# plai-group/latent-flexible-video-diffusion-modeling

Hardware: NVIDIA B200
Metric: denoiser frame-steps/sec (sampling) (higher is better)
Workload: dtype bf16

## Files before the change

### include/fdm_b200.h

```cpp
#ifndef FDM_B200_H_
#define FDM_B200_H_

#include <stddef.h>
#include <stdint.h>

#ifdef __cplusplus
extern "C" {
#endif

#define FDM_ABI_VERSION 2

enum { FDM_F32 = 0, FDM_BF16 = 1 };

enum {
  FDM_OK = 0,
  FDM_ERR_BAD_ARG = -1,
  FDM_ERR_UNSUPPORTED = -2,
  FDM_ERR_CUDA = -3,
  FDM_ERR_NO_DEVICE = -4
};

int fdm_abi_version(void);
const char* fdm_status_string(int status);
const char* fdm_last_cuda_error(void);
// ... 18 lines not shown
  const float* bias;
  const float* resid;
  float* y_f32;
  void* y_op;
  double* stats;
  int32_t N, Hin, Win, C0, C1, Cout;
  int32_t ksize, stride, upsample;
  int32_t a_dtype, op_dtype, out_nchw, engine;
  int32_t resid_norm;
  int32_t rn_T;
  float rn_eps;
  const float* rn_tstats;
  const double* rn_stats;
  const float* rn_gamma;
  const float* rn_beta;
} fdm_conv_args;
int fdm_conv(const fdm_conv_args* a, void* stream);

typedef struct {
  const void* xa;
  const float* xb;
  const double* stats_a;
  const double* stats_b;
  const float* gamma;
  const float* beta;
  const float* film;
  void* out_op;
  float* out_f32;
  void* raw_op;
  int32_t N, HW, Ca, Cb, T;
// ... 337 lines not shown
```

### latent-flexible-video-diffusion-modeling_b200/csrc/conv_simt.cu

```cuda
#include "common.cuh"

namespace fdm {

constexpr int BM = 64, BN = 64, BK = 16, NT = 256;

struct ConvParams {
  const void* a0;
  const float* w0;
  const void* a1;
  const float* w1;
  const float* bias;
  const float* resid;
  float* y_f32;
  void* y_op;
  double* stats;
  int N, Hin, Win, C0, C1, Cout, Ho, Wo;
  int ksize, stride, upsample, out_nchw;
  int M;
};

template <typename AT, typename OT>
__global__ void __launch_bounds__(NT) conv_simt_kernel(ConvParams p) {
  pdl_wait();
  __shared__ __align__(16) float As[BK][BM + 4];
// ... 202 lines not shown
  return check_launch();
}

}

extern "C" int fdm_conv(const fdm_conv_args* a, void* stream) {
  using namespace fdm;
  FDM_REQUIRE(a != nullptr && a->a0 != nullptr && a->w0 != nullptr, FDM_ERR_BAD_ARG);
  FDM_REQUIRE(a->N > 0 && a->Hin > 0 && a->Win > 0 && a->C0 > 0 && a->Cout > 0, FDM_ERR_BAD_ARG);
  FDM_REQUIRE(a->ksize == 1 || a->ksize == 3, FDM_ERR_UNSUPPORTED);
  FDM_REQUIRE(a->stride == 1 || a->stride == 2, FDM_ERR_UNSUPPORTED);
  FDM_REQUIRE(!(a->upsample && a->stride != 1), FDM_ERR_UNSUPPORTED);
  FDM_REQUIRE((a->a1 == nullptr) == (a->w1 == nullptr), FDM_ERR_BAD_ARG);
  FDM_REQUIRE(a->y_f32 != nullptr || a->y_op != nullptr, FDM_ERR_BAD_ARG);
  FDM_REQUIRE(!(a->out_nchw && a->y_f32 == nullptr), FDM_ERR_BAD_ARG);
  cudaStream_t st = reinterpret_cast<cudaStream_t>(stream);
  if (a->engine == FDM_CONV_TC) {
    if (a->out_nchw && a->ksize == 3) {
      const int rh = conv_head_launch(a, st);
      if (rh != FDM_ERR_UNSUPPORTED) return rh;
    }
    const int rc = (a->ksize == 3 || a->C0 >= 256) ? conv_halo_launch(a, st) : FDM_ERR_UNSUPPORTED;
    return rc == FDM_ERR_UNSUPPORTED ? conv_tc_launch(a, st) : rc;
  }
  if (a->engine == FDM_CONV_TC_TAP) return conv_tc_launch(a, st);
  FDM_REQUIRE(a->engine == FDM_CONV_SIMT, FDM_ERR_BAD_ARG);
  FDM_REQUIRE(a->resid_norm == 0, FDM_ERR_UNSUPPORTED);
  return conv_simt_launch(a, st);
}
```

### latent-flexible-video-diffusion-modeling_b200/csrc/conv_tc.cu

```cuda
#include "tc_common.cuh"
#include <mutex>

namespace fdm {

constexpr int TC_BM = 128;
constexpr int TC_BK = 64;
constexpr int TC_THREADS = 192;
constexpr int A_TILE_BYTES = TC_BM * TC_BK * 2;

struct TcParams {
  const float* bias;
  const float* resid;
  float* y_f32;
  __nv_bfloat16* y_op;
  double* stats;
  int M, HWo, Wo, Ho, Cout;
  int wbox, hbox, nbox;
  int taps, ksize, pad, stride;
  int kchunks0, kchunks1;
  int klast0, klast1;
  int out_nchw;
  int stages;
  int nr;
  int a_slot;
  int stage_bytes;
  int resid_norm, rn_T;
  float rn_eps;
  double rn_inv_cnt;
  const float* rn_tstats;
  const double* rn_stats;
  const float* rn_gamma;
  const float* rn_beta;
};

constexpr int TC_MAX_STAGES = 8;
constexpr int TC_STG_ROW = 36;

template <int BN>
struct TcSmem {
  static constexpr int B_TILE_BYTES = BN * TC_BK * 2;
  static constexpr int STAGE_BYTES = A_TILE_BYTES + B_TILE_BYTES;
  static constexpr int TMEM_COLS = BN < 32 ? 32 : BN;
  static constexpr int EXTRA_BYTES = 1024;
  static_assert(STAGE_BYTES >= 4 * 32 * TC_STG_ROW * 4, "one stage must hold the epilogue staging");
};

template <int BN, bool RN>
__global__ void __launch_bounds__(TC_THREADS, RN ? 3 : 0) conv_tc_kernel(const __grid_constant__ CUtensorMap ta0,
                                                            const __grid_constant__ CUtensorMap tw0,
                                                            const __grid_constant__ CUtensorMap ta1,
                                                            const __grid_constant__ CUtensorMap tw1, const TcParams p) {
  using S = TcSmem<BN>;
  extern __shared__ uint8_t smem_raw[];
  uint8_t* smem = reinterpret_cast<uint8_t*>((reinterpret_cast<uintptr_t>(smem_raw) + 1023) & ~uintptr_t(1023));
  __shared__ __align__(8) uint64_t full_bar[TC_MAX_STAGES];
  __shared__ __align__(8) uint64_t empty_bar[TC_MAX_STAGES];
  __shared__ __align__(8) uint64_t tmem_full_bar;
  __shared__ uint32_t tmem_base_slot;
  __shared__ __align__(16) float4 rn_tab[RN ? 4 : 1][2][2][RN ? 32 : 1];

  const int warp = threadIdx.x >> 5, lane = threadIdx.x & 31;
  const int mt = blockIdx.x, n_off = blockIdx.y * BN;
  const int m0 = mt * TC_BM;
  const int iters0 = (p.taps / p.nr) * p.kchunks0;
  const int iters = iters0 + p.kchunks1;
  const int stages = p.stages;
  constexpr int B_TAP_BYTES = BN * 128;

  if (warp == 0 && lane == 0) {
    asm volatile("prefetch.tensormap [%0];" ::"l"(&ta0) : "memory");
    asm volatile("prefetch.tensormap [%0];" ::"l"(&tw0) : "memory");
    if (p.kchunks1) {
      asm volatile("prefetch.tensormap [%0];" ::"l"(&ta1) : "memory");
      asm volatile("prefetch.tensormap [%0];" ::"l"(&tw1) : "memory");
// ... 93 lines not shown
        }
        umma_commit(&empty_bar[stage]);
        }
        __syncwarp();
        if (++stage == stages) { stage = 0; phase ^= 1; }
      }
      if (elect_one_sync()) umma_commit(&tmem_full_bar);
      __syncwarp();
    }
  } else {
    const int g = warp & 3;
    float* stg = reinterpret_cast<float*>(smem) + g * 32 * TC_STG_ROW;
    const int sub = lane >> 3, cq = (lane & 7) * 4;
    const int m_w = m0 + g * 32;
    const bool two_frames = p.HWo < 32;
    int rn_n[2] = {0, 0}, rn_b[2] = {0, 0};
    if (RN) {
      rn_n[0] = min(m_w, p.M - 1) / p.HWo;
      rn_n[1] = two_frames ? min(m_w + 16, p.M - 1) / p.HWo : rn_n[0];
      rn_b[0] = rn_n[0] / p.rn_T;
      rn_b[1] = rn_n[1] / p.rn_T;
      if (p.resid_norm == 3) {
        const int col = n_off + 4 * lane;
#pragma unroll
        for (int hh = 0; hh < 2; ++hh) {
          float4 mu = make_float4(0.f, 0.f, 0.f, 0.f), ad = mu;
          if ((hh == 0 || two_frames) && col < p.Cout && 4 * lane < BN && m_w + hh * 16 < p.M) {
            const float4 gm = __ldg(reinterpret_cast<const float4*>(p.rn_gamma + col));
            const float4 bt = __ldg(reinterpret_cast<const float4*>(p.rn_beta + col));
            const double2* st = reinterpret_cast<const double2*>(p.rn_stats + ((size_t)rn_n[hh] * p.Cout + col) * 2);
            const double2 s0 = st[0], s1_ = st[1], s2_ = st[2], s3 = st[3];
            const double mean = (s0.x + s1_.x + s2_.x + s3.x) * p.rn_inv_cnt;
            const double var = fmax((s0.y + s1_.y + s2_.y + s3.y) * p.rn_inv_cnt - mean * mean, 0.0);
            const float mf = (float)mean, rs = rsqrtf((float)var + p.rn_eps);
            mu = make_float4(gm.x * rs, gm.y * rs, gm.z * rs, gm.w * rs);
            ad = make_float4(bt.x - mf * mu.x, bt.y - mf * mu.y, bt.z - mf * mu.z, bt.w - mf * mu.w);
          }
          rn_tab[g][hh][0][lane] = mu;
          rn_tab[g][hh][1][lane] = ad;
        }
        __syncwarp();
      }
    }
    mbar_wait(&tmem_full_bar, 0);
    tcgen05_fence_after();
    const bool direct = BN >= 32 && p.y_f32 == nullptr && p.y_op != nullptr && p.resid == nullptr && p.stats == nullptr &&
                        !p.out_nchw && (p.Cout & 31) == 0;
#pragma unroll 1
    for (int c = 0; c < BN; c += 32) {
      uint32_t v[32];
      tmem_ld_32x32b_x32(tmem_base + ((uint32_t)(g * 32) << 16) + c, v);
      if (direct) {
        uint8_t* sb = reinterpret_cast<uint8_t*>(stg);
        const bool cols_ok = n_off + c < p.Cout;
#pragma unroll
        for (int q = 0; q < 32; q += 8) {
          float4 b0 = make_float4(0.f, 0.f, 0.f, 0.f), b1 = b0;
          if (p.bias != nullptr && cols_ok) {
            b0 = __ldg(reinterpret_cast<const float4*>(p.bias + n_off + c + q));
            b1 = __ldg(reinterpret_cast<const float4*>(p.bias + n_off + c + q + 4));
          }
// ... 70 lines not shown
            const int grp = (c + cq) >> 2;
#pragma unroll
            for (int hh = 0; hh < 2; ++hh) {
              const float4 mu = rn_tab[g][two_frames ? hh : 0][0][grp], ad = rn_tab[g][two_frames ? hh : 0][1][grp];
#pragma unroll
              for (int i = 4 * hh; i < 4 * hh + 4; ++i) {
                res[i].x = fmaf(res[i].x, mu.x, ad.x);
                res[i].y = fmaf(res[i].y, mu.y, ad.y);
                res[i].z = fmaf(res[i].z, mu.z, ad.z);
                res[i].w = fmaf(res[i].w, mu.w, ad.w);
              }
            }
          }
        }
        float s1[2][4], s2[2][4];
#pragma unroll
        for (int hh = 0; hh < 2; ++hh)
#pragma unroll
          for (int q = 0; q < 4; ++q) s1[hh][q] = s2[hh][q] = 0.f;
#pragma unroll
        for (int i = 0; i < 8; ++i) {
          const int row = i * 4 + sub;
          const int m = m_w + row;
          const float4 a = *reinterpret_cast<const float4*>(stg + row * TC_STG_ROW + cq);
          const float o[4] = {a.x + bias.x + res[i].x, a.y + bias.y + res[i].y, a.z + bias.z + res[i].z, a.w + bias.w + res[i].w};
          if (m < p.M && col_ok) {
#pragma unroll
            for (int q = 0; q < 4; ++q) { s1[i >> 2][q] += o[q]; s2[i >> 2][q] = fmaf(o[q], o[q], s2[i >> 2][q]); }
            const size_t off = (size_t)m * p.Cout + col;
            if (p.y_f32 != nullptr) *reinterpret_cast<float4*>(p.y_f32 + off) = make_float4(o[0], o[1], o[2], o[3]);
            if (p.y_op != nullptr) OpType<__nv_bfloat16>::store4(p.y_op + off, make_float4(o[0], o[1], o[2], o[3]));
          }
        }
        if (p.stats != nullptr) {
#pragma unroll
          for (int hh = 0; hh < 2; ++hh)
#pragma unroll
            for (int q = 0; q < 4; ++q) {
              s1[hh][q] += __shfl_xor_sync(0xffffffffu, s1[hh][q], 8);
              s2[hh][q] += __shfl_xor_sync(0xffffffffu, s2[hh][q], 8);
              s1[hh][q] += __shfl_xor_sync(0xffffffffu, s1[hh][q], 16);
              s2[hh][q] += __shfl_xor_sync(0xffffffffu, s2[hh][q], 16);
            }
          if (sub == 0 && col_ok) {
            if (two_frames) {
#pragma unroll
// ... 2 lines not shown
                if (mseg < p.M) {
                  double* dst = p.stats + ((size_t)(mseg / p.HWo) * p.Cout + col) * 2;
#pragma unroll
                  for (int q = 0; q < 4; ++q) {
                    atomicAdd(dst + 2 * q, (double)s1[hh][q]);
                    atomicAdd(dst + 2 * q + 1, (double)s2[hh][q]);
                  }
                }
              }
            } else if (m_w < p.M) {
              double* dst = p.stats + ((size_t)(m_w / p.HWo) * p.Cout + col) * 2;
#pragma unroll
              for (int q = 0; q < 4; ++q) {
                atomicAdd(dst + 2 * q, (double)(s1[0][q] + s1[1][q]));
                atomicAdd(dst + 2 * q + 1, (double)(s2[0][q] + s2[1][q]));
              }
            }
          }
        }
      }
      __syncwarp();
    }
  }
  tcgen05_fence_before();
  __syncthreads();
  if (warp == 2) {
    tcgen05_fence_after();
    asm volatile("tcgen05.dealloc.cta_group::1.sync.aligned.b32 %0, %1;" ::"r"(tmem_base), "n"(S::TMEM_COLS));
  }
}
// ... 21 lines not shown
  return enc(m, CU_TENSOR_MAP_DATA_TYPE_BFLOAT16, 4, const_cast<void*>(ptr), dims, strides, box, estr, CU_TENSOR_MAP_INTERLEAVE_NONE,
             CU_TENSOR_MAP_SWIZZLE_128B, CU_TENSOR_MAP_L2_PROMOTION_L2_128B, CU_TENSOR_MAP_FLOAT_OOB_FILL_NONE) == CUDA_SUCCESS;
}

static bool encode_w(CUtensorMap* m, const void* ptr, int taps, int co_pad, int ci_pad, int bn, int box_taps) {
  EncodeTiledFn enc = get_tensormap_encoder();
  if (!enc) return false;
  cuuint64_t dims[3] = {(cuuint64_t)ci_pad, (cuuint64_t)co_pad, (cuuint64_t)taps};
  cuuint64_t strides[2] = {(cuuint64_t)ci_pad * 2, (cuuint64_t)co_pad * ci_pad * 2};
  cuuint32_t box[3] = {(cuuint32_t)TC_BK, (cuuint32_t)bn, (cuuint32_t)box_taps};
  cuuint32_t estr[3] = {1, 1, 1};
  return enc(m, CU_TENSOR_MAP_DATA_TYPE_BFLOAT16, 3, const_cast<void*>(ptr), dims, strides, box, estr, CU_TENSOR_MAP_INTERLEAVE_NONE,
             CU_TENSOR_MAP_SWIZZLE_128B, CU_TENSOR_MAP_L2_PROMOTION_L2_256B, CU_TENSOR_MAP_FLOAT_OOB_FILL_NONE) == CUDA_SUCCESS;
}

template <int BN, bool RN = false>
static int launch_tc(const CUtensorMap& ta0, const CUtensorMap& tw0, const CUtensorMap& ta1, const CUtensorMap& tw1,
                     TcParams& p, cudaStream_t st) {
  using S = TcSmem<BN>;
  constexpr int SMEM_MAX = (RN ? 216 : 226) * 1024;
  static std::once_flag once;
  static cudaError_t attr_err = cudaSuccess;
  std::call_once(once, [] {
    attr_err = cudaFuncSetAttribute(conv_tc_kernel<BN, RN>, cudaFuncAttributeMaxDynamicSharedMemorySize, SMEM_MAX);
  });
  if (attr_err != cudaSuccess) {
    set_last_error(attr_err);
    return FDM_ERR_CUDA;
  }
  dim3 grid((p.M + TC_BM - 1) / TC_BM, (p.Cout + BN - 1) / BN);
  const int budget = (long)grid.x * grid.y <= 148 ? SMEM_MAX : SMEM_MAX / 2;
  p.a_slot = p.nr * A_TILE_BYTES;
  p.stage_bytes = p.nr * S::STAGE_BYTES;
  int stages = (budget - S::EXTRA_BYTES) / p.stage_bytes;
  const int iters = (p.taps / p.nr) * p.kchunks0 + p.kchunks1;
  if (stages > TC_MAX_STAGES) stages = TC_MAX_STAGES;
  if (stages > iters) stages = iters;
  if (stages < 1) return FDM_ERR_UNSUPPORTED;
  p.stages = stages;
  fdm::launch(conv_tc_kernel<BN, RN>, dim3(grid), dim3(TC_THREADS), stages * p.stage_bytes + S::EXTRA_BYTES, st, ta0, tw0, ta1, tw1, p);
  return check_launch();
}

static inline int round_up(int v, int m) { return (v + m - 1) / m * m; }

int conv_tc_launch(const fdm_conv_args* a, cudaStream_t st) {
  FDM_REQUIRE(a->a_dtype == FDM_BF16, FDM_ERR_UNSUPPORTED);
  FDM_REQUIRE(!a->upsample, FDM_ERR_UNSUPPORTED);
  FDM_REQUIRE(a->C0 % 8 == 0 && (a->a1 == nullptr || a->C1 % 8 == 0), FDM_ERR_UNSUPPORTED);
  if (a->out_nchw) {
    FDM_REQUIRE(a->y_f32 != nullptr && a->y_op == nullptr && a->resid == nullptr && a->stats == nullptr, FDM_ERR_UNSUPPORTED);
  } else {
    FDM_REQUIRE(a->Cout % 4 == 0, FDM_ERR_UNSUPPORTED);
  }
  FDM_REQUIRE(a->y_op == nullptr || a->op_dtype == FDM_BF16, FDM_ERR_UNSUPPORTED);
// ... 17 lines not shown
  p.taps = a->ksize * a->ksize; p.ksize = a->ksize; p.pad = pad; p.stride = a->stride;
  p.kchunks0 = (a->C0 + TC_BK - 1) / TC_BK;
  p.kchunks1 = a->a1 ? (a->C1 + TC_BK - 1) / TC_BK : 0;
  p.klast0 = (a->C0 - (p.kchunks0 - 1) * TC_BK + 15) / 16;
  p.klast1 = a->a1 ? (a->C1 - (p.kchunks1 - 1) * TC_BK + 15) / 16 : 0;
  p.out_nchw = a->out_nchw;
  p.resid_norm = a->resid_norm; p.rn_T = a->rn_T > 0 ? a->rn_T : 1; p.rn_eps = a->rn_eps;
  p.rn_inv_cnt = 1.0 / (4.0 * (double)HWo);
  p.rn_tstats = a->rn_tstats; p.rn_stats = a->rn_stats; p.rn_gamma = a->rn_gamma; p.rn_beta = a->rn_beta;
  if (a->resid_norm != 0) {
    FDM_REQUIRE(a->resid_norm == 2 || a->resid_norm == 3, FDM_ERR_BAD_ARG);
    FDM_REQUIRE(a->resid != nullptr && a->rn_gamma != nullptr && a->rn_beta != nullptr, FDM_ERR_BAD_ARG);
    FDM_REQUIRE(a->resid_norm == 2 ? a->rn_tstats != nullptr : a->rn_stats != nullptr, FDM_ERR_BAD_ARG);
    FDM_REQUIRE(a->Cout == 128 && a->ksize == 1 && !a->out_nchw && (HWo % 32 == 0 || HWo == 16), FDM_ERR_UNSUPPORTED);
  }
  int bn = a->Cout % 128 == 0 ? 128 : (a->Cout >= 64 ? 64 : (a->Cout > 16 ? 32 : 16));
  const int mtiles = (p.M + TC_BM - 1) / TC_BM;
  const int cta_cap = (a->ksize == 1 && a->C0 <= 128 && a->a1 == nullptr) ? 3 * 148 : 148;
  while (bn > 32 && mtiles * ((a->Cout + bn / 2 - 1) / (bn / 2)) <= cta_cap) bn >>= 1;
  const int co_pad = round_up(a->Cout, 16);
  const long ctas = (long)mtiles * ((a->Cout + bn - 1) / bn);
  p.nr = (a->ksize == 3 && ctas <= 148) ? 3 : 1;
  CUtensorMap ta0, tw0, ta1, tw1;
  bool ok = encode_act(&ta0, a->a0, a->N, a->Hin, a->Win, a->C0, p.wbox, p.hbox, p.nbox, a->stride) &&
            encode_w(&tw0, a->w0, p.taps, co_pad, round_up(a->C0, TC_BK), bn, p.nr);
  if (ok && a->a1) {
    ok = encode_act(&ta1, a->a1, a->N, Ho, Wo, a->C1, p.wbox, p.hbox, p.nbox, 1) &&
         encode_w(&tw1, a->w1, 1, co_pad, round_up(a->C1, TC_BK), bn, 1);
  } else {
    ta1 = ta0;
    tw1 = tw0;
  }
  FDM_REQUIRE(ok, FDM_ERR_UNSUPPORTED);
  if (p.resid_norm != 0) {
    if (bn == 128) return launch_tc<128, true>(ta0, tw0, ta1, tw1, p, st);
    if (bn == 64) return launch_tc<64, true>(ta0, tw0, ta1, tw1, p, st);
    return launch_tc<32, true>(ta0, tw0, ta1, tw1, p, st);
  }
  if (bn == 128) return launch_tc<128>(ta0, tw0, ta1, tw1, p, st);
  if (bn == 64) return launch_tc<64>(ta0, tw0, ta1, tw1, p, st);
  if (bn == 32) return launch_tc<32>(ta0, tw0, ta1, tw1, p, st);
  return launch_tc<16>(ta0, tw0, ta1, tw1, p, st);
}

}
```

### latent-flexible-video-diffusion-modeling_b200/improved_diffusion/_native.py

```python
import ctypes as C
import os

_HERE = os.path.dirname(os.path.abspath(__file__))
LIB_PATH = os.path.join(os.path.dirname(_HERE), "libfdm_sm100.so")

F32, BF16 = 0, 1
CONV_SIMT, CONV_TC, CONV_TC_TAP = 0, 1, 2

vp, i32, i64, f32 = C.c_void_p, C.c_int32, C.c_int64, C.c_float


def _S(name, fields):
    return type(name, (C.Structure,), {"_fields_": fields})


InputPrepArgs = _S("InputPrepArgs", [("x", vp), ("x0", vp), ("obs_mask", vp), ("xin", vp), ("xin_bf16", vp),
                                     ("N", i32), ("C", i32), ("H", i32), ("W", i32), ("Cpad", i32)])
ConvArgs = _S("ConvArgs", [("a0", vp), ("w0", vp), ("a1", vp), ("w1", vp), ("bias", vp), ("resid", vp),
                           ("y_f32", vp), ("y_op", vp), ("stats", vp),
                           ("N", i32), ("Hin", i32), ("Win", i32), ("C0", i32), ("C1", i32), ("Cout", i32),
                           ("ksize", i32), ("stride", i32), ("upsample", i32),
                           ("a_dtype", i32), ("op_dtype", i32), ("out_nchw", i32), ("engine", i32),
                           ("resid_norm", i32), ("rn_T", i32), ("rn_eps", f32), ("rn_tstats", vp), ("rn_stats", vp),
                           ("rn_gamma", vp), ("rn_beta", vp)])
GnApplyArgs = _S("GnApplyArgs", [("xa", vp), ("xb", vp), ("stats_a", vp), ("stats_b", vp), ("gamma", vp), ("beta", vp),
                                 ("film", vp), ("out_op", vp), ("out_f32", vp), ("raw_op", vp),
                                 ("N", i32), ("HW", i32), ("Ca", i32), ("Cb", i32), ("T", i32),
                                 ("film_stride", i32), ("film_off", i32), ("silu", i32), ("op_dtype", i32), ("eps", f32),
                                 ("xa_bf16", i32), ("film_add", i32), ("drop_philox", vp), ("drop_p", f32), ("drop_salt", i32)])
TemporalGnArgs = _S("TemporalGnArgs", [("x", vp), ("gamma", vp), ("beta", vp), ("out_f32", vp), ("out_op", vp),
                                       ("B", i32), ("T", i32), ("HW", i32), ("C", i32), ("op_dtype", i32), ("eps", f32)])
TimestepEmbeddingArgs = _S("TimestepEmbeddingArgs", [("t", vp), ("t_index", vp), ("t_table", vp), ("freqs", vp), ("out", vp),
                                                     ("B", i32), ("dim", i32)])
LinearProblem = _S("LinearProblem", [("x", vp), ("w", vp), ("b", vp), ("y", vp),
                                     ("M", i32), ("K", i32), ("Nout", i32), ("ldx", i32), ("ldy", i32), ("silu_in", i32)])
GroupedLinearArgs = _S("GroupedLinearArgs", [("problems", vp), ("count", i32), ("max_M", i32), ("max_Nout", i32), ("max_K", i32)])
RpeHiddenProblem = _S("RpeHiddenProblem", [("wd", vp), ("bd", vp), ("hidden", vp), ("C", i32), ("te_off", i32)])
RpeHiddenArgs = _S("RpeHiddenArgs", [("te", vp), ("frame_indices", vp), ("problems", vp),
                                     ("B", i32), ("T", i32), ("te_stride", i32), ("count", i32), ("max_C", i32),
# ... 153 lines not shown
```

### latent-flexible-video-diffusion-modeling_b200/improved_diffusion/engine.py

```python
import ctypes as C
import os

import torch as th
import torch.nn as nn

from . import _native as N_
from .nn import timestep_freqs


class NativeShapeError(RuntimeError):
    pass


class Buf:
    __slots__ = ("name", "nbytes", "offset", "first", "last", "persistent", "arena")

    def __init__(self, name, nbytes, persistent=False, arena="main"):
        self.name, self.nbytes, self.persistent, self.arena = name, (int(nbytes) + 255) // 256 * 256, persistent, arena
        self.offset, self.first, self.last = None, None, None


class Plan:
    def __init__(self, engine, B, T, H, W):
        self.engine, self.B, self.T, self.H, self.W = engine, B, T, H, W
# ... 855 lines not shown

        stem_tc = self.use_tc and self.tc_ok(8, 0, m.model_channels, 3, 1, 0, H, W) and Cin <= 8
        if stem_tc:
            xin = P.buf("xin", Nf * H * W * 8 * 2)
            P.op("fdm_input_prep", N_.InputPrepArgs, x=P.x, x0=P.x0, obs_mask=P.obs, xin=None, xin_bf16=xin, N=Nf, C=Cin - 1,
                 H=H, W=W, Cpad=8)
        else:
            xin = P.buf("xin", Nf * H * W * Cin * 4)
            P.op("fdm_input_prep", N_.InputPrepArgs, x=P.x, x0=P.x0, obs_mask=P.obs, xin=xin, xin_bf16=None, N=Nf, C=Cin - 1,
                 H=H, W=W, Cpad=0)

        class Act:
            def __init__(s, buf, st, Cc, Hh, Ww):
                s.buf, s.st, s.C, s.H, s.W, s.op = buf, st, Cc, Hh, Ww, None
                s.biases = ()

        def with_op_copy(act):
            act.op = P.buf("act_op", Nf * act.H * act.W * act.C * osz)
            return act.op

        def new_act(name, Cc, Hh, Ww):
            return Act(P.buf(name, Nf * Hh * Ww * Cc * 4), P.stats(name, Nf, Cc), Cc, Hh, Ww)

        def res_block(rb, xa, xb=None, want_op=False):
            Hh, Ww = xa.H, xa.W
            Ci = xa.C + (xb.C if xb else 0)
            Co = rb.out_channels
            hw = Hh * Ww
            has_skip = not isinstance(rb.skip_connection, nn.Identity)
            a1 = P.buf("res_a1", Nf * hw * Ci * osz)
            raw = P.buf("res_raw", Nf * hw * Ci * osz) if has_skip else None
            gn, c1 = rb.in_layers[0], rb.in_layers[2]
            P.op("fdm_gn_apply", N_.GnApplyArgs, xa=xa.buf, xb=xb.buf if xb else None, stats_a=xa.st,
                 stats_b=xb.st if xb else None, gamma=f32(gn.weight), beta=f32(gn.bias), film=None, out_op=a1, out_f32=None,
                 raw_op=raw, N=Nf, HW=hw, Ca=xa.C, Cb=xb.C if xb else 0, T=T, film_stride=0, film_off=0, silu=1,
                 op_dtype=opd, eps=gn.eps)
            h1_bf16 = self.use_tc and not train
            if h1_bf16:
                h1_ = Act(P.buf("res_h1_op", Nf * hw * Co * osz), P.stats("res_h1", Nf, Co), Co, Hh, Ww)
                conv(a1, Ci, Hh, Ww, c1.weight, Co, 3, bias=f32(c1.bias), y_op=h1_.buf, stats=h1_.st)
            else:
                h1_ = new_act("res_h1", Co, Hh, Ww)
                conv(a1, Ci, Hh, Ww, c1.weight, Co, 3, bias=f32(c1.bias), y_f32=h1_.buf, stats=h1_.st)
            h1_.biases = (c1.bias,)
            gn2, c2 = rb.out_layers[0], rb.out_layers[3]
            a2 = P.buf("res_a2", Nf * hw * Co * osz)
            P.res_a2.append((a2, Co, Hh, Ww))
            dropf = dict(drop_philox=P.drop_philox, drop_p=P.drop_p, drop_salt=len(P.res_a2)) if P.drop_philox is not None else {}
            P.op("fdm_gn_apply", N_.GnApplyArgs, xa=h1_.buf, xb=None, stats_a=h1_.st, stats_b=None, gamma=f32(gn2.weight),
                 beta=f32(gn2.bias), film=cond, out_op=a2, out_f32=None, raw_op=None, N=Nf, HW=hw, Ca=Co, Cb=0, T=T,
                 film_stride=cond_cols, film_off=film_off[id(rb)], silu=1, op_dtype=opd, eps=gn2.eps, xa_bf16=1 if h1_bf16 else 0,
                 film_add=0 if m.use_scale_shift_norm else 1, **dropf)
            out = new_act("res_out", Co, Hh, Ww)
            yop = with_op_copy(out) if want_op else None
            sk = rb.skip_connection
            out.biases = (c2.bias, sk.bias) if has_skip else (c2.bias,)
            if has_skip:
                if sk.kernel_size != (1, 1):
                    raise NotImplementedError("ResBlock(use_conv=True) 3x3 skip is never built by create_model")
                conv(a2, Co, Hh, Ww, c2.weight, Co, 3, a1=raw, C1=Ci, w1=sk.weight, bias=bias_sum(c2.bias, sk.bias),
                     y_f32=out.buf, y_op=yop, stats=out.st)
            else:
                conv(a2, Co, Hh, Ww, c2.weight, Co, 3, bias=f32(c2.bias), resid=xa.buf, y_f32=out.buf, y_op=yop, stats=out.st)

            def bwd():
                g_out = gact(out)
                go = get_op(out)
                da2 = P.buf("d_a2", Nf * hw * Co * osz)
                dgrad(go, Co, Hh, Ww, c2.weight, Co, 3, out_op=da2)
                draw = None
                if has_skip:
                    wgrad(a2, opd, Co, Co, Hh, Ww, go, Co, 3, 1, c2.weight)
                    draw = P.buf("d_raw", Nf * hw * Ci * osz)
                    dgrad(go, Co, Hh, Ww, sk.weight, Ci, 1, out_op=draw)
                    wgrad(raw, opd, Ci, Ci, Hh, Ww, go, Co, 1, 1, sk.weight)
                else:
                    wgrad(a2, opd, Co, Co, Hh, Ww, go, Co, 3, 1, c2.weight)
                gn_bwd(h1_, None, gn2, film_off[id(rb)], da2, None, None, 1, last=True, dropf=dropf)
# ... 78 lines not shown
                conv(yn_op, Cc, Hh, Ww, sa.qkv.weight, 3 * Cc, 1, bias=f32(sa.qkv.bias), y_op=qkv2)
            o2 = P.buf("sa_o", Nf * hw * Cc * osz)
            P.flops += 4 * hw * hw * Cc * Nf
            sa_lse = P.buf("sa_lse", Nf * sa.num_heads * hw * 4) if (train and self.use_tc) else None
            P.op("fdm_attn_spatial", N_.AttnSpatialArgs, qkv=qkv2, out=o2, N=Nf, L=hw, C=Cc, heads=sa.num_heads,
                 qkv_dtype=opd, out_dtype=opd, engine=0 if self.use_tc else 1, lse=sa_lse, attn_mean=s_mean)
            z = new_act("sa_z", Cc, Hh, Ww)
            z.biases = (sa.proj_out.bias,)
            if s_fused:
                conv(o2, Cc, Hh, Ww, sa.proj_out.weight, Cc, 1, bias=f32(sa.proj_out.bias), resid=y.buf, y_f32=z.buf,
                     y_op=with_op_copy(z) if want_op else None, stats=z.st, resid_norm=3, rn_eps=sa.norm.eps, rn_stats=y.st,
                     rn_gamma=f32(sa.norm.weight), rn_beta=f32(sa.norm.bias))
            else:
                conv(o2, Cc, Hh, Ww, sa.proj_out.weight, Cc, 1, bias=f32(sa.proj_out.bias), resid=yn, y_f32=z.buf,
                     y_op=with_op_copy(z) if want_op else None, stats=z.st)

            def bwd():
                n_tok = Nf * hw
                g_z = gact(z)
                gz = get_op(z)
                do2 = P.buf("d_sa_o", n_tok * Cc * osz)
                dgrad(gz, Cc, Hh, Ww, sa.proj_out.weight, Cc, 1, out_op=do2)
                wgrad(o2, opd, Cc, Cc, Hh, Ww, gz, Cc, 1, 1, sa.proj_out.weight)
                dqkv2 = P.buf("d_sa_qkv", n_tok * 3 * Cc * osz)
                P.bflops += 10 * hw * hw * Cc * Nf
                P.op("fdm_attn_spatial_bwd", N_.AttnSpatialBwdArgs, qkv=qkv2, out=o2, dout=do2, dqkv=dqkv2,
                     lse=sa_lse if sa_lse is not None else P.at_lse, dsum=P.at_dsum, N=Nf, L=hw, C=Cc, heads=sa.num_heads,
                     dtype=opd, lse_from_forward=1 if sa_lse is not None else 0)
                P.at_rows = max(P.at_rows, Nf * sa.num_heads * hw)
                dyn = P.buf("d_sa_yn", n_tok * Cc * osz)
# ... 28 lines not shown
            out = new_act("down" if down else "up", x.C, Ho, Wo)
            out.biases = (cv.bias,)
            Hc, Wc = (x.H, x.W) if down else (Ho, Wo)
            a = None
            if not down and not train and self.up_tc_ok(x.C, x.H, x.W):
                a = x.op
                if a is None:
                    a = P.buf("resample_a", Nf * x.H * x.W * x.C * osz)
                    P.op("fdm_cast", N_.CastArgs, x=x.buf, out=a, N=Nf, H=x.H, W=x.W, C=x.C, upsample=0, op_dtype=opd, colsum=None,
                         colsum2=None)
                conv(a, x.C, x.H, x.W, cv.weight, x.C, 3, upsample=1, bias=f32(cv.bias), y_f32=out.buf, stats=out.st,
                     y_op=with_op_copy(out) if want_op else None)
            elif (self.use_tc and self.tc_ok(x.C, 0, x.C, 3, 2 if down else 1, 0, Ho, Wo)) or (train and not down):
                if down and x.op is not None:
                    a = x.op
                else:
                    a = P.buf("resample_a", Nf * Hc * Wc * x.C * osz)
                    P.op("fdm_cast", N_.CastArgs, x=x.buf, out=a, N=Nf, H=x.H, W=x.W, C=x.C, upsample=0 if down else 1,
                         op_dtype=opd, colsum=None, colsum2=None)
                conv(a, x.C, Hc, Wc, cv.weight, x.C, 3, stride=2 if down else 1, bias=f32(cv.bias), y_f32=out.buf,
                     stats=out.st, y_op=with_op_copy(out) if (want_op and not train) else None)
            else:
                conv(x.buf, x.C, x.H, x.W, cv.weight, x.C, 3, stride=2 if down else 1, upsample=0 if down else 1,
                     bias=f32(cv.bias), y_f32=out.buf, stats=out.st, a_dtype=N_.F32)

            def bwd():
                Cc = x.C
                g_out = gact(out)
                go = get_op(out)
                if down:
                    z_ = to_op(g_out, Cc, Ho, Wo, up=2)
                    gx = gact(x)
                    dgrad(z_, Cc, Hc, Wc, cv.weight, Cc, 3, out_f32=gx, resid=gx if acc(x) else None)
                    if self.use_tc and a is not None:
                        wgrad(a, opd, Cc, Cc, Hc, Wc, z_, Cc, 3, 1, cv.weight)
                    else:
# ... 50 lines not shown
                elif isinstance(layer, Downsample):
                    h = resample(layer, h, True, want_op=want_op)
                elif isinstance(layer, Upsample):
                    h = resample(layer, h, False, want_op=want_op)
                else:
                    raise NotImplementedError(type(layer))
                P.taps[names[id(layer)]] = (h.buf, h.C, h.H, h.W)
            return h

        h, hs = None, []
        in_stages = list(m.input_blocks)
        for si, stage in enumerate(in_stages):
            nxt = in_stages[si + 1] if si + 1 < len(in_stages) else None
            feeds = nxt is not None and len(nxt) == 1 and isinstance(nxt[0], Downsample)
            h = run_stage(stage, h, feeds_downsample=feeds)
            hs.append(h)
        h = run_stage(m.middle_block, h)
        for stage in m.output_blocks:
            h = run_stage(stage, h, hs.pop())
        gn, cv = m.out[0], m.out[2]
        a = P.buf("head_a", Nf * H * W * h.C * osz)
        P.op("fdm_gn_apply", N_.GnApplyArgs, xa=h.buf, xb=None, stats_a=h.st, stats_b=None, gamma=f32(gn.weight),
             beta=f32(gn.bias), film=None, out_op=a, out_f32=None, raw_op=None, N=Nf, HW=H * W, Ca=h.C, Cb=0, T=T,
             film_stride=0, film_off=0, silu=1, op_dtype=opd, eps=gn.eps)
        conv(a, h.C, H, W, cv.weight, m.out_channels, 3, bias=f32(cv.bias), y_f32=P.eps, out_nchw=1)

        if train:
            h_last, head_a, Co_ = h, a, m.out_channels
            P.geps = P.buf("geps", Nf * Co_ * H * W * 4, True)
            P.at_rows = 1
# ... 166 lines not shown
```

Before: 94680.

## Fuse GroupNorm+FiLM+SiLU and nearest upsample into tensor-core conv epilogue

Adds an epilogue mode to the tcgen05 conv kernel that computes per-frame GroupNorm statistics in-register (32 groups, Cout 128, 4x4 or 8x8 spatial), applies gamma/beta with optional FiLM scale-shift and SiLU, and writes the bf16 operand directly, optionally replicated 2x2 for nearest upsampling. The engine routes the ResBlock's first conv, and producers feeding a following GroupNorm or upsample, through this fused path. This removes separate gn_apply and cast kernels and the f32 or bf16 intermediate round trips on small-resolution layers. In exchange it uses more shared memory and named barriers and supports only narrow shape constraints. It also drops the stats atomics when the output is not needed as a skip.

```diff
diff --git a/include/fdm_b200.h b/include/fdm_b200.h
--- a/include/fdm_b200.h
+++ b/include/fdm_b200.h
@@ -56,6 +56,12 @@
   const double* rn_stats;
   const float* rn_gamma;
   const float* rn_beta;
+  int32_t out_gn, og_silu, og_T, op_upsample;
+  float og_eps;
+  int32_t og_film_stride, og_film_off;
+  const float* og_gamma;
+  const float* og_beta;
+  const float* og_film;
 } fdm_conv_args;
 int fdm_conv(const fdm_conv_args* a, void* stream);
 
diff --git a/latent-flexible-video-diffusion-modeling_b200/csrc/conv_simt.cu b/latent-flexible-video-diffusion-modeling_b200/csrc/conv_simt.cu
--- a/latent-flexible-video-diffusion-modeling_b200/csrc/conv_simt.cu
+++ b/latent-flexible-video-diffusion-modeling_b200/csrc/conv_simt.cu
@@ -240,7 +240,24 @@
   FDM_REQUIRE((a->a1 == nullptr) == (a->w1 == nullptr), FDM_ERR_BAD_ARG);
   FDM_REQUIRE(a->y_f32 != nullptr || a->y_op != nullptr, FDM_ERR_BAD_ARG);
   FDM_REQUIRE(!(a->out_nchw && a->y_f32 == nullptr), FDM_ERR_BAD_ARG);
+  FDM_REQUIRE((a->out_gn == 0 || a->out_gn == 1) && (a->op_upsample == 0 || a->op_upsample == 1), FDM_ERR_BAD_ARG);
+  if (a->out_gn) {
+    FDM_REQUIRE(a->y_op != nullptr && a->og_gamma != nullptr && a->og_beta != nullptr, FDM_ERR_BAD_ARG);
+    FDM_REQUIRE(a->og_eps >= 0.f && (a->og_silu == 0 || a->og_silu == 1), FDM_ERR_BAD_ARG);
+    if (a->og_film != nullptr) {
+      FDM_REQUIRE(a->og_T > 0 && a->og_film_off >= 0 && a->og_film_off + 2 * a->Cout <= a->og_film_stride, FDM_ERR_BAD_ARG);
+      FDM_REQUIRE(a->og_film_off % 4 == 0 && a->og_film_stride % 4 == 0 && (reinterpret_cast<uintptr_t>(a->og_film) & 15) == 0,
+                  FDM_ERR_UNSUPPORTED);
+    }
+    FDM_REQUIRE(((reinterpret_cast<uintptr_t>(a->og_gamma) | reinterpret_cast<uintptr_t>(a->og_beta)) & 15) == 0,
+                FDM_ERR_UNSUPPORTED);
+  }
+  FDM_REQUIRE(!a->op_upsample || a->y_op != nullptr, FDM_ERR_BAD_ARG);
   cudaStream_t st = reinterpret_cast<cudaStream_t>(stream);
+  if (a->out_gn || a->op_upsample) {
+    FDM_REQUIRE(a->engine == FDM_CONV_TC || a->engine == FDM_CONV_TC_TAP, FDM_ERR_UNSUPPORTED);
+    return conv_tc_launch(a, st);
+  }
   if (a->engine == FDM_CONV_TC) {
     if (a->out_nchw && a->ksize == 3) {
       const int rh = conv_head_launch(a, st);
diff --git a/latent-flexible-video-diffusion-modeling_b200/csrc/conv_tc.cu b/latent-flexible-video-diffusion-modeling_b200/csrc/conv_tc.cu
--- a/latent-flexible-video-diffusion-modeling_b200/csrc/conv_tc.cu
+++ b/latent-flexible-video-diffusion-modeling_b200/csrc/conv_tc.cu
@@ -31,6 +31,13 @@
   const double* rn_stats;
   const float* rn_gamma;
   const float* rn_beta;
+  int og_mode, og_silu, og_up, og_T;
+  float og_eps;
+  float og_inv_cnt;
+  const float* og_gamma;
+  const float* og_beta;
+  const float* og_film;
+  int og_film_stride, og_film_off;
 };
 
 constexpr int TC_MAX_STAGES = 8;
@@ -45,7 +52,7 @@
   static_assert(STAGE_BYTES >= 4 * 32 * TC_STG_ROW * 4, "one stage must hold the epilogue staging");
 };
 
-template <int BN, bool RN>
+template <int BN, bool RN, bool OG = false>
 __global__ void __launch_bounds__(TC_THREADS, RN ? 3 : 0) conv_tc_kernel(const __grid_constant__ CUtensorMap ta0,
                                                             const __grid_constant__ CUtensorMap tw0,
                                                             const __grid_constant__ CUtensorMap ta1,
@@ -58,6 +65,7 @@
   __shared__ __align__(8) uint64_t tmem_full_bar;
   __shared__ uint32_t tmem_base_slot;
   __shared__ __align__(16) float4 rn_tab[RN ? 4 : 1][2][2][RN ? 32 : 1];
+  __shared__ __align__(16) float4 og_coef[OG ? 4 : 1][2][2][OG ? 32 : 1];
 
   const int warp = threadIdx.x >> 5, lane = threadIdx.x & 31;
   const int mt = blockIdx.x, n_off = blockIdx.y * BN;
@@ -181,6 +189,34 @@
     const int sub = lane >> 3, cq = (lane & 7) * 4;
     const int m_w = m0 + g * 32;
     const bool two_frames = p.HWo < 32;
+    if constexpr (OG) {
+      if (p.og_mode) {
+        int og_b[2];
+        og_b[0] = min(m_w, p.M - 1) / p.HWo / p.og_T;
+        og_b[1] = two_frames ? min(m_w + 16, p.M - 1) / p.HWo / p.og_T : og_b[0];
+        const int col = n_off + 4 * lane;
+#pragma unroll
+        for (int hh = 0; hh < 2; ++hh) {
+          float4 G = make_float4(0.f, 0.f, 0.f, 0.f), Bc = G;
+          if ((hh == 0 || two_frames) && 4 * lane < BN) {
+            const float4 gm = __ldg(reinterpret_cast<const float4*>(p.og_gamma + col));
+            const float4 bt = __ldg(reinterpret_cast<const float4*>(p.og_beta + col));
+            float4 sc = make_float4(1.f, 1.f, 1.f, 1.f), sh = make_float4(0.f, 0.f, 0.f, 0.f);
+            if (p.og_film != nullptr) {
+              const float* f = p.og_film + (size_t)og_b[hh] * p.og_film_stride + p.og_film_off;
+              const float4 fs = __ldg(reinterpret_cast<const float4*>(f + col));
+              sh = __ldg(reinterpret_cast<const float4*>(f + p.Cout + col));
+              sc = make_float4(1.f + fs.x, 1.f + fs.y, 1.f + fs.z, 1.f + fs.w);
+            }
+            G = make_float4(gm.x * sc.x, gm.y * sc.y, gm.z * sc.z, gm.w * sc.w);
+            Bc = make_float4(fmaf(bt.x, sc.x, sh.x), fmaf(bt.y, sc.y, sh.y), fmaf(bt.z, sc.z, sh.z), fmaf(bt.w, sc.w, sh.w));
+          }
+          og_coef[g][hh][0][lane] = G;
+          og_coef[g][hh][1][lane] = Bc;
+        }
+        __syncwarp();
+      }
+    }
     int rn_n[2] = {0, 0}, rn_b[2] = {0, 0};
     if (RN) {
       rn_n[0] = min(m_w, p.M - 1) / p.HWo;
@@ -211,7 +247,7 @@
     }
     mbar_wait(&tmem_full_bar, 0);
     tcgen05_fence_after();
-    const bool direct = BN >= 32 && p.y_f32 == nullptr && p.y_op != nullptr && p.resid == nullptr && p.stats == nullptr &&
+    const bool direct = !OG && BN >= 32 && p.y_f32 == nullptr && p.y_op != nullptr && p.resid == nullptr && p.stats == nullptr &&
                         !p.out_nchw && (p.Cout & 31) == 0;
 #pragma unroll 1
     for (int c = 0; c < BN; c += 32) {
@@ -312,6 +348,7 @@
           }
         }
         float s1[2][4], s2[2][4];
+        float4 ov[OG ? 8 : 1];
 #pragma unroll
         for (int hh = 0; hh < 2; ++hh)
 #pragma unroll
@@ -322,12 +359,13 @@
           const int m = m_w + row;
           const float4 a = *reinterpret_cast<const float4*>(stg + row * TC_STG_ROW + cq);
           const float o[4] = {a.x + bias.x + res[i].x, a.y + bias.y + res[i].y, a.z + bias.z + res[i].z, a.w + bias.w + res[i].w};
+          if constexpr (OG) ov[i] = make_float4(o[0], o[1], o[2], o[3]);
           if (m < p.M && col_ok) {
 #pragma unroll
             for (int q = 0; q < 4; ++q) { s1[i >> 2][q] += o[q]; s2[i >> 2][q] = fmaf(o[q], o[q], s2[i >> 2][q]); }
             const size_t off = (size_t)m * p.Cout + col;
             if (p.y_f32 != nullptr) *reinterpret_cast<float4*>(p.y_f32 + off) = make_float4(o[0], o[1], o[2], o[3]);
-            if (p.y_op != nullptr) OpType<__nv_bfloat16>::store4(p.y_op + off, make_float4(o[0], o[1], o[2], o[3]));
+            if (!OG && p.y_op != nullptr) OpType<__nv_bfloat16>::store4(p.y_op + off, make_float4(o[0], o[1], o[2], o[3]));
           }
         }
         if (p.stats != nullptr) {
@@ -360,6 +398,86 @@
               for (int q = 0; q < 4; ++q) {
                 atomicAdd(dst + 2 * q, (double)(s1[0][q] + s1[1][q]));
                 atomicAdd(dst + 2 * q + 1, (double)(s2[0][q] + s2[1][q]));
+              }
+            }
+          }
+        }
+        if constexpr (OG) {
+          __shared__ float2 og_tab[2][4][8];
+          float mean_o[2] = {0.f, 0.f}, m2_o[2] = {0.f, 0.f};
+          if (p.og_mode) {
+            float mean[2], m2[2];
+#pragma unroll
+            for (int hh = 0; hh < 2; ++hh) {
+              float s = 0.f;
+#pragma unroll
+              for (int i = 4 * hh; i < 4 * hh + 4; ++i) s += (ov[i].x + ov[i].y) + (ov[i].z + ov[i].w);
+              s += __shfl_xor_sync(0xffffffffu, s, 8);
+              s += __shfl_xor_sync(0xffffffffu, s, 16);
+              mean[hh] = s;
+            }
+            if (two_frames) {
+              mean[0] *= 1.f / 64.f;
+              mean[1] *= 1.f / 64.f;
+            } else {
+              mean[0] = mean[1] = (mean[0] + mean[1]) * (1.f / 128.f);
+            }
+#pragma unroll
+            for (int hh = 0; hh < 2; ++hh) {
+              float d = 0.f;
+#pragma unroll
+              for (int i = 4 * hh; i < 4 * hh + 4; ++i) {
+                const float dx = ov[i].x - mean[hh], dy = ov[i].y - mean[hh], dz = ov[i].z - mean[hh], dw = ov[i].w - mean[hh];
+                d = fmaf(dx, dx, fmaf(dy, dy, fmaf(dz, dz, fmaf(dw, dw, d))));
+              }
+              d += __shfl_xor_sync(0xffffffffu, d, 8);
+              d += __shfl_xor_sync(0xffffffffu, d, 16);
+              m2[hh] = d;
+            }
+            if (!two_frames) {
+              const int par = (c >> 5) & 1;
+              const float m2w = m2[0] + m2[1];
+              if (sub == 0) og_tab[par][g][lane] = make_float2(mean[0], m2w);
+              if (g >> 1) asm volatile("bar.sync 2, 64;" ::: "memory");
+              else asm volatile("bar.sync 1, 64;" ::: "memory");
+              const float2 other = og_tab[par][g ^ 1][lane & 7];
+              const float dm = mean[0] - other.x;
+              mean[0] = mean[1] = 0.5f * (mean[0] + other.x);
+              m2[0] = m2[1] = (m2w + other.y) + dm * dm * 64.f;
+            }
+            mean_o[0] = mean[0]; mean_o[1] = mean[1];
+            m2_o[0] = m2[0]; m2_o[1] = m2[1];
+          }
+          const int col = n_off + c + cq;
+#pragma unroll
+          for (int hh = 0; hh < 2; ++hh) {
+            float4 mu = make_float4(1.f, 1.f, 1.f, 1.f), ad = make_float4(0.f, 0.f, 0.f, 0.f);
+            if (p.og_mode) {
+              const int grp = (c + cq) >> 2, th = two_frames ? hh : 0;
+              const float4 G = og_coef[g][th][0][grp], Bc = og_coef[g][th][1][grp];
+              const float rs = rsqrtf(m2_o[hh] * p.og_inv_cnt + p.og_eps), nm = -mean_o[hh];
+              mu = make_float4(G.x * rs, G.y * rs, G.z * rs, G.w * rs);
+              ad = make_float4(fmaf(nm, mu.x, Bc.x), fmaf(nm, mu.y, Bc.y), fmaf(nm, mu.z, Bc.z), fmaf(nm, mu.w, Bc.w));
+            }
+#pragma unroll
+            for (int i = 4 * hh; i < 4 * hh + 4; ++i) {
+              const int m = m_w + i * 4 + sub;
+              if (m >= p.M) continue;
+              float4 v = ov[i];
+              if (p.og_mode) {
+                v = make_float4(fmaf(v.x, mu.x, ad.x), fmaf(v.y, mu.y, ad.y), fmaf(v.z, mu.z, ad.z), fmaf(v.w, mu.w, ad.w));
+                if (p.og_silu) v = make_float4(silu_f(v.x), silu_f(v.y), silu_f(v.z), silu_f(v.w));
+              }
+              if (p.og_up) {
+                const int f = m / p.HWo, r = m - f * p.HWo, oh = r / p.Wo, ow = r - oh * p.Wo;
+                const size_t row = (size_t)2 * p.Wo * p.Cout;
+                __nv_bfloat16* d = p.y_op + ((size_t)(f * 2 * p.Ho + 2 * oh) * 2 * p.Wo + 2 * ow) * p.Cout + col;
+                OpType<__nv_bfloat16>::store4(d, v);
+                OpType<__nv_bfloat16>::store4(d + p.Cout, v);
+                OpType<__nv_bfloat16>::store4(d + row, v);
+                OpType<__nv_bfloat16>::store4(d + row + p.Cout, v);
+              } else {
+                OpType<__nv_bfloat16>::store4(p.y_op + (size_t)m * p.Cout + col, v);
               }
             }
           }
@@ -411,15 +529,15 @@
              CU_TENSOR_MAP_SWIZZLE_128B, CU_TENSOR_MAP_L2_PROMOTION_L2_256B, CU_TENSOR_MAP_FLOAT_OOB_FILL_NONE) == CUDA_SUCCESS;
 }
 
-template <int BN, bool RN = false>
+template <int BN, bool RN = false, bool OG = false>
 static int launch_tc(const CUtensorMap& ta0, const CUtensorMap& tw0, const CUtensorMap& ta1, const CUtensorMap& tw1,
                      TcParams& p, cudaStream_t st) {
   using S = TcSmem<BN>;
-  constexpr int SMEM_MAX = (RN ? 216 : 226) * 1024;
+  constexpr int SMEM_MAX = (RN && OG ? 208 : RN || OG ? 216 : 226) * 1024;
   static std::once_flag once;
   static cudaError_t attr_err = cudaSuccess;
   std::call_once(once, [] {
-    attr_err = cudaFuncSetAttribute(conv_tc_kernel<BN, RN>, cudaFuncAttributeMaxDynamicSharedMemorySize, SMEM_MAX);
+    attr_err = cudaFuncSetAttribute(conv_tc_kernel<BN, RN, OG>, cudaFuncAttributeMaxDynamicSharedMemorySize, SMEM_MAX);
   });
   if (attr_err != cudaSuccess) {
     set_last_error(attr_err);
@@ -435,7 +553,7 @@
   if (stages > iters) stages = iters;
   if (stages < 1) return FDM_ERR_UNSUPPORTED;
   p.stages = stages;
-  fdm::launch(conv_tc_kernel<BN, RN>, dim3(grid), dim3(TC_THREADS), stages * p.stage_bytes + S::EXTRA_BYTES, st, ta0, tw0, ta1, tw1, p);
+  fdm::launch(conv_tc_kernel<BN, RN, OG>, dim3(grid), dim3(TC_THREADS), stages * p.stage_bytes + S::EXTRA_BYTES, st, ta0, tw0, ta1, tw1, p);
   return check_launch();
 }
 
@@ -483,6 +601,12 @@
     FDM_REQUIRE(a->resid_norm == 2 ? a->rn_tstats != nullptr : a->rn_stats != nullptr, FDM_ERR_BAD_ARG);
     FDM_REQUIRE(a->Cout == 128 && a->ksize == 1 && !a->out_nchw && (HWo % 32 == 0 || HWo == 16), FDM_ERR_UNSUPPORTED);
   }
+  const bool og = a->out_gn || a->op_upsample;
+  if (og) FDM_REQUIRE(a->Cout == 128 && (HWo == 16 || HWo == 64) && !a->out_nchw, FDM_ERR_UNSUPPORTED);
+  p.og_mode = a->out_gn; p.og_silu = a->og_silu; p.og_up = a->op_upsample; p.og_T = a->og_T > 0 ? a->og_T : 1;
+  p.og_eps = a->og_eps; p.og_inv_cnt = 1.f / (4.f * (float)HWo);
+  p.og_gamma = a->og_gamma; p.og_beta = a->og_beta; p.og_film = a->og_film;
+  p.og_film_stride = a->og_film_stride; p.og_film_off = a->og_film_off;
   int bn = a->Cout % 128 == 0 ? 128 : (a->Cout >= 64 ? 64 : (a->Cout > 16 ? 32 : 16));
   const int mtiles = (p.M + TC_BM - 1) / TC_BM;
   const int cta_cap = (a->ksize == 1 && a->C0 <= 128 && a->a1 == nullptr) ? 3 * 148 : 148;
@@ -501,6 +625,16 @@
     tw1 = tw0;
   }
   FDM_REQUIRE(ok, FDM_ERR_UNSUPPORTED);
+  if (og) {
+    if (p.resid_norm != 0) {
+      if (bn == 128) return launch_tc<128, true, true>(ta0, tw0, ta1, tw1, p, st);
+      if (bn == 64) return launch_tc<64, true, true>(ta0, tw0, ta1, tw1, p, st);
+      return launch_tc<32, true, true>(ta0, tw0, ta1, tw1, p, st);
+    }
+    if (bn == 128) return launch_tc<128, false, true>(ta0, tw0, ta1, tw1, p, st);
+    if (bn == 64) return launch_tc<64, false, true>(ta0, tw0, ta1, tw1, p, st);
+    return launch_tc<32, false, true>(ta0, tw0, ta1, tw1, p, st);
+  }
   if (p.resid_norm != 0) {
     if (bn == 128) return launch_tc<128, true>(ta0, tw0, ta1, tw1, p, st);
     if (bn == 64) return launch_tc<64, true>(ta0, tw0, ta1, tw1, p, st);
diff --git a/latent-flexible-video-diffusion-modeling_b200/improved_diffusion/_native.py b/latent-flexible-video-diffusion-modeling_b200/improved_diffusion/_native.py
--- a/latent-flexible-video-diffusion-modeling_b200/improved_diffusion/_native.py
+++ b/latent-flexible-video-diffusion-modeling_b200/improved_diffusion/_native.py
@@ -22,7 +22,9 @@
                            ("ksize", i32), ("stride", i32), ("upsample", i32),
                            ("a_dtype", i32), ("op_dtype", i32), ("out_nchw", i32), ("engine", i32),
                            ("resid_norm", i32), ("rn_T", i32), ("rn_eps", f32), ("rn_tstats", vp), ("rn_stats", vp),
-                           ("rn_gamma", vp), ("rn_beta", vp)])
+                           ("rn_gamma", vp), ("rn_beta", vp),
+                           ("out_gn", i32), ("og_silu", i32), ("og_T", i32), ("op_upsample", i32), ("og_eps", f32),
+                           ("og_film_stride", i32), ("og_film_off", i32), ("og_gamma", vp), ("og_beta", vp), ("og_film", vp)])
 GnApplyArgs = _S("GnApplyArgs", [("xa", vp), ("xb", vp), ("stats_a", vp), ("stats_b", vp), ("gamma", vp), ("beta", vp),
                                  ("film", vp), ("out_op", vp), ("out_f32", vp), ("raw_op", vp),
                                  ("N", i32), ("HW", i32), ("Ca", i32), ("Cb", i32), ("T", i32),
diff --git a/latent-flexible-video-diffusion-modeling_b200/improved_diffusion/engine.py b/latent-flexible-video-diffusion-modeling_b200/improved_diffusion/engine.py
--- a/latent-flexible-video-diffusion-modeling_b200/improved_diffusion/engine.py
+++ b/latent-flexible-video-diffusion-modeling_b200/improved_diffusion/engine.py
@@ -893,6 +893,22 @@
             def __init__(s, buf, st, Cc, Hh, Ww):
                 s.buf, s.st, s.C, s.H, s.W, s.op = buf, st, Cc, Hh, Ww, None
                 s.biases = ()
+                s.prod = None
+                s.skip = False
+
+        def out_gn_ok(Cc, Hh, Ww):
+            return self.use_tc and not train and m.use_scale_shift_norm and Cc == 128 and Hh * Ww in (16, 64)
+
+        def producer(act):
+            fields = P.ops[-1][2]
+            if fields["y_op"] is None and fields["engine"] == N_.CONV_TC and out_gn_ok(act.C, act.H, act.W):
+                act.prod = (len(P.ops) - 1, fields)
+
+        def into_producer(act, buf, **fields):
+            idx, f = act.prod
+            f.update(y_op=buf, **fields)
+            buf.first = buf.last = idx
+            act.prod = None
 
         def with_op_copy(act):
             act.op = P.buf("act_op", Nf * act.H * act.W * act.C * osz)
@@ -910,26 +926,37 @@
             a1 = P.buf("res_a1", Nf * hw * Ci * osz)
             raw = P.buf("res_raw", Nf * hw * Ci * osz) if has_skip else None
             gn, c1 = rb.in_layers[0], rb.in_layers[2]
-            P.op("fdm_gn_apply", N_.GnApplyArgs, xa=xa.buf, xb=xb.buf if xb else None, stats_a=xa.st,
-                 stats_b=xb.st if xb else None, gamma=f32(gn.weight), beta=f32(gn.bias), film=None, out_op=a1, out_f32=None,
-                 raw_op=raw, N=Nf, HW=hw, Ca=xa.C, Cb=xb.C if xb else 0, T=T, film_stride=0, film_off=0, silu=1,
-                 op_dtype=opd, eps=gn.eps)
+            if xb is None and xa.prod is not None and gn.num_groups == 32:
+                into_producer(xa, a1, out_gn=1, og_silu=1, og_eps=gn.eps, og_gamma=f32(gn.weight), og_beta=f32(gn.bias))
+                if not xa.skip:
+                    P.ops[a1.first][2]["stats"] = None
+            else:
+                P.op("fdm_gn_apply", N_.GnApplyArgs, xa=xa.buf, xb=xb.buf if xb else None, stats_a=xa.st,
+                     stats_b=xb.st if xb else None, gamma=f32(gn.weight), beta=f32(gn.bias), film=None, out_op=a1, out_f32=None,
+                     raw_op=raw, N=Nf, HW=hw, Ca=xa.C, Cb=xb.C if xb else 0, T=T, film_stride=0, film_off=0, silu=1,
+                     op_dtype=opd, eps=gn.eps)
             h1_bf16 = self.use_tc and not train
-            if h1_bf16:
-                h1_ = Act(P.buf("res_h1_op", Nf * hw * Co * osz), P.stats("res_h1", Nf, Co), Co, Hh, Ww)
-                conv(a1, Ci, Hh, Ww, c1.weight, Co, 3, bias=f32(c1.bias), y_op=h1_.buf, stats=h1_.st)
-            else:
-                h1_ = new_act("res_h1", Co, Hh, Ww)
-                conv(a1, Ci, Hh, Ww, c1.weight, Co, 3, bias=f32(c1.bias), y_f32=h1_.buf, stats=h1_.st)
-            h1_.biases = (c1.bias,)
             gn2, c2 = rb.out_layers[0], rb.out_layers[3]
             a2 = P.buf("res_a2", Nf * hw * Co * osz)
             P.res_a2.append((a2, Co, Hh, Ww))
-            dropf = dict(drop_philox=P.drop_philox, drop_p=P.drop_p, drop_salt=len(P.res_a2)) if P.drop_philox is not None else {}
-            P.op("fdm_gn_apply", N_.GnApplyArgs, xa=h1_.buf, xb=None, stats_a=h1_.st, stats_b=None, gamma=f32(gn2.weight),
-                 beta=f32(gn2.bias), film=cond, out_op=a2, out_f32=None, raw_op=None, N=Nf, HW=hw, Ca=Co, Cb=0, T=T,
-                 film_stride=cond_cols, film_off=film_off[id(rb)], silu=1, op_dtype=opd, eps=gn2.eps, xa_bf16=1 if h1_bf16 else 0,
-                 film_add=0 if m.use_scale_shift_norm else 1, **dropf)
+            if out_gn_ok(Co, Hh, Ww) and gn2.num_groups == 32:
+                h1_ = None
+                conv(a1, Ci, Hh, Ww, c1.weight, Co, 3, bias=f32(c1.bias), y_op=a2, out_gn=1, og_silu=1, og_T=T, og_eps=gn2.eps,
+                     og_gamma=f32(gn2.weight), og_beta=f32(gn2.bias), og_film=cond, og_film_stride=cond_cols,
+                     og_film_off=film_off[id(rb)])
+            else:
+                if h1_bf16:
+                    h1_ = Act(P.buf("res_h1_op", Nf * hw * Co * osz), P.stats("res_h1", Nf, Co), Co, Hh, Ww)
+                    conv(a1, Ci, Hh, Ww, c1.weight, Co, 3, bias=f32(c1.bias), y_op=h1_.buf, stats=h1_.st)
+                else:
+                    h1_ = new_act("res_h1", Co, Hh, Ww)
+                    conv(a1, Ci, Hh, Ww, c1.weight, Co, 3, bias=f32(c1.bias), y_f32=h1_.buf, stats=h1_.st)
+                h1_.biases = (c1.bias,)
+                dropf = dict(drop_philox=P.drop_philox, drop_p=P.drop_p, drop_salt=len(P.res_a2)) if P.drop_philox is not None else {}
+                P.op("fdm_gn_apply", N_.GnApplyArgs, xa=h1_.buf, xb=None, stats_a=h1_.st, stats_b=None, gamma=f32(gn2.weight),
+                     beta=f32(gn2.bias), film=cond, out_op=a2, out_f32=None, raw_op=None, N=Nf, HW=hw, Ca=Co, Cb=0, T=T,
+                     film_stride=cond_cols, film_off=film_off[id(rb)], silu=1, op_dtype=opd, eps=gn2.eps,
+                     xa_bf16=1 if h1_bf16 else 0, film_add=0 if m.use_scale_shift_norm else 1, **dropf)
             out = new_act("res_out", Co, Hh, Ww)
             yop = with_op_copy(out) if want_op else None
             sk = rb.skip_connection
@@ -941,6 +968,7 @@
                      y_f32=out.buf, y_op=yop, stats=out.st)
             else:
                 conv(a2, Co, Hh, Ww, c2.weight, Co, 3, bias=f32(c2.bias), resid=xa.buf, y_f32=out.buf, y_op=yop, stats=out.st)
+            producer(out)
 
             def bwd():
                 g_out = gact(out)
@@ -1049,6 +1077,7 @@
             else:
                 conv(o2, Cc, Hh, Ww, sa.proj_out.weight, Cc, 1, bias=f32(sa.proj_out.bias), resid=yn, y_f32=z.buf,
                      y_op=with_op_copy(z) if want_op else None, stats=z.st)
+            producer(z)
 
             def bwd():
                 n_tok = Nf * hw
@@ -1107,12 +1136,16 @@
             elif (self.use_tc and self.tc_ok(x.C, 0, x.C, 3, 2 if down else 1, 0, Ho, Wo)) or (train and not down):
                 if down and x.op is not None:
                     a = x.op
+                elif not down and x.prod is not None:
+                    a = P.buf("resample_a", Nf * Hc * Wc * x.C * osz)
+                    into_producer(x, a, op_upsample=1)
                 else:
                     a = P.buf("resample_a", Nf * Hc * Wc * x.C * osz)
                     P.op("fdm_cast", N_.CastArgs, x=x.buf, out=a, N=Nf, H=x.H, W=x.W, C=x.C, upsample=0 if down else 1,
                          op_dtype=opd, colsum=None, colsum2=None)
                 conv(a, x.C, Hc, Wc, cv.weight, x.C, 3, stride=2 if down else 1, bias=f32(cv.bias), y_f32=out.buf,
                      stats=out.st, y_op=with_op_copy(out) if (want_op and not train) else None)
+                producer(out)
             else:
                 conv(x.buf, x.C, x.H, x.W, cv.weight, x.C, 3, stride=2 if down else 1, upsample=0 if down else 1,
                      bias=f32(cv.bias), y_f32=out.buf, stats=out.st, a_dtype=N_.F32)
@@ -1193,6 +1226,7 @@
             nxt = in_stages[si + 1] if si + 1 < len(in_stages) else None
             feeds = nxt is not None and len(nxt) == 1 and isinstance(nxt[0], Downsample)
             h = run_stage(stage, h, feeds_downsample=feeds)
+            h.skip = True
             hs.append(h)
         h = run_stage(m.middle_block, h)
         for stage in m.output_blocks:
```

New measurement: 95440, median of 6. About the same (+0.8%).
